# mklarqvist/StormBitmaps

Hardware: AMD Instinct MI355X
Metric: 64-bit bitmap words/s, XX^T upper-tri pairwise AND+popcount (10000x65536) (higher is better)
Workload: dtype u64 (bits as exact FP4 0/1 MFMA operands, f32 accumulate < 2^24); 1 GPU; STORM_contiguous_t N=10000 M=65536 dense draws=32768 seed=42 (BASELINE configs[1], README `benchmark 65536 10000`); entry_point=storm_hip_pairw_dense_launch == STORM_contig_pairw_intersect_cardinality_blocked, kernel_variant=4, work_items=13688

## Files before the change

### stormbitmaps_amd/csrc/storm_hip.hip

```cpp
#include "storm_hip_internal.h"

#include <chrono>

#include <algorithm>
#include <atomic>
#include <cstdarg>
#include <cstdlib>
#include <cstring>

namespace storm {

static thread_local char g_error[512] = "";

void set_error(const char* fmt, ...) {
    va_list ap;
    va_start(ap, fmt);
    vsnprintf(g_error, sizeof(g_error), fmt, ap);
    va_end(ap);
}

#define STORM_PAIR(A, B)                 \
    "v_and_b32 %[t], %[" A "], %[" B "]\n\t" \
    "s_nop 0\n\t"                        \
    "v_bcnt_u32_b32 %[acc], %[t], %[acc]\n\t"
// ... 605 lines not shown
        {"k2_max_run", &C::k2_max_run, RANGE, 0, 4096, 0, {},
         "k2_max_run out of range (0 = chosen by the list-scheduling estimate, 1..4096)"},
        {"k2_ring", &C::k2_ring, HOOK, 0, 0, 0, {}, nullptr, {}, nullptr, set_ring},
        {"k2_shadow_budget_mb", &C::k2_shadow_budget_mb, RANGE, 0, 1 << 22, 0, {}, "k2_shadow_budget_mb must be 0 (unbounded) .. 4194304",
         {}, nullptr, nullptr, drop_shadow},
        {"k2_tile_shape", &C::k2_tile_shape, SET, 0, 0, 0, {0, 1, 2, 3, 4, 5, 6, 16, 32},
         "k2_tile_shape must be 0 (chosen by the matrix), 5 (both operands as FP4 images in the LDS, 16x16x128 MFMAs), 1, 2 (bit operands inflated in registers), 3 / 4 (B as FP4 images in the LDS, 16x16x128 / 32x32x64 MFMAs), 6 (128 x 128 tiles, k-parts whose sums meet inside the launch), 16 or 32 (FP4 shadow)",
         {1, 16},
         "k2_tile_shape = 1 / 16 (tilebits_kernel, tile16_fp4_kernel) is a form of the tools build (`make probes`), not of the shipped library"},
        {"k2_ring_sync", &C::k2_ring_sync, BOOL},
        {"k2_wave_below", &C::k2_wave_below, RANGE, 0, 1 << 30, 0, {}, "k2_wave_below: 0 (never) .. 2^30 tiles of 256 x 256"},
        {"k2_part_slots", &C::k2_part_slots, RANGE, 0, 2, 0, {}, "k2_part_slots must be 0 (by the length of the segments), 1 or 2 per CU"},
        {"k2_part_min_chunks", &C::k2_part_min_chunks, RANGE, 1, 4096, 0, {}, "k2_part_min_chunks: 1 .. 4096 chunks of 512 bits"},
        {"k2_part_narrow", &C::k2_part_narrow, BOOL},
        {"k2_part_cost_diag", &C::k2_part_cost_diag, RANGE, 10, 100, 0, {}, "k2_part_cost_diag: 10 .. 100 percent of a full tile's chunk"},
        {"k2_ring_cost_diag", &C::k2_ring_cost_diag, RANGE, 5, 100, 0, {}, kCostText},
        {"k2_ring_cost_ragged", &C::k2_ring_cost_ragged, RANGE, 5, 100, 0, {}, kCostText},
        {"k2_tile_cost_diag", &C::k2_tile_cost_diag, RANGE, 5, 100, 0, {}, kCostText},
        {"k2_tile_cost_ragged", &C::k2_tile_cost_ragged, RANGE, 5, 100, 0, {}, kCostText},
        {"k2_strip_operands", &C::k2_strip_operands, RANGE, 0, 6, 0, {},
         "k2_strip_operands must be 0 (by size), 1 (bit operands, one item per workgroup), 2 (bit operands, one stream per workgroup), 3 (the same with a ring per wave), 4 (FP4 shadow), 5 (bit operands, FP4 image built in the LDS) or 6 (the same with 512-row A tiles, two halves behind one image)",
         {1, 3},
         "k2_strip_operands = 1 (stripbits_kernel) and 3 (bitwave_kernel) are forms of the tools build (`make probes`), not of the shipped library"},
        {"k2_shard_pairs", &C::k2_shard_pairs, BOOL},
        {"k2_matrix_pad", &C::k2_matrix_pad, HOOK, 0, 0, 0, {}, nullptr, {}, nullptr, set_matrix_pad},
        {"k2_fold_inline", &C::k2_fold_inline, HOOK, 0, 0, 0, {}, nullptr, {}, nullptr, set_fold_inline},
        {"k2_wave_ring", &C::k2_wave_ring, SET, 0, 0, 0, {0, 3, 4, 6, 8}, "k2_wave_ring must be 0 (by occupancy), 3, 4, 6 or 8"},
        {"k2_stream_max_rows", &C::k2_stream_max_rows, RANGE, 0, 1ll << 31, 0, {}, "k2_stream_max_rows must be 0 .. 2^31"},
        {"k2_stream_groups_per_cu", &C::k2_stream_groups_per_cu, RANGE, 0, 255, 0, {}, "k2_stream_groups_per_cu must be 0 (auto) .. 255"},
        {"k2_stream_min_piece", &C::k2_stream_min_piece, RANGE, 1, 4096, 0, {}, "%s must be 1..4096 stages"},
        {"k2_stream_min_run", &C::k2_stream_min_run, RANGE, 1, 4096, 0, {}, "%s must be 1..4096 stages"},
        {"k2_stream_w3_1", &C::k2_stream_w3_1, RANGE, 10, 1000, 0, {}, "%s must be 10..1000 percent of the first workgroup's share"},
        {"k2_stream_w3_2", &C::k2_stream_w3_2, RANGE, 10, 1000, 0, {}, "%s must be 10..1000 percent of the first workgroup's share"},
        {"k2_shape", &C::k2_shape, SET, 0, 0, 0, {16, 32}, "k2_shape must be 16 (16x16x128 MFMA) or 32 (32x32x64)", {32},
         "k2_shape = 32 (strip_fp4_kernel) is a form of the tools build (`make probes`), not of the shipped library"},
        {"keep_shadow", &C::keep_shadow, BOOL, 0, 0, 0, {}, nullptr, {}, nullptr, nullptr, drop_shadow},
        {"k2_matrix_parts", &C::k2_matrix_parts, BOOL},
        {"k2_matrix_min_part", &C::k2_matrix_min_part, RANGE, 4, 4096, 4, {},
         "k2_matrix_min_part: a multiple of 4 in 4 .. 4096 (stages of 128 bits)"},
        {"k2_matrix_split", &C::k2_matrix_split, BOOL},
        {"k2_pitch_pad", &C::k2_pitch_pad, RANGE, -1, 65536, 128, {}, "k2_pitch_pad must be -1 (auto) or a multiple of 128 in 0..65536"},
        {"k2_lds_pad", &C::k2_lds_pad, RANGE, 0, 120 * 1024, 0, {}, "k2_lds_pad must be 0..122880"},
        {"k2_persistent", &C::k2_persistent, BOOL, 0, 0, 0, {}, nullptr, {1},
         "k2_persistent (strip_fp4_kernel with work queues) is a form of the tools build (`make probes`), not of the shipped library"},
        {"k2_lpt_rounds", &C::k2_lpt_rounds, RANGE, 0, 63, 0, {}, "k2_lpt_rounds must be 0..63"},
        {"k2_tail_slices", &C::k2_tail_slices, RANGE, 0, 255, 0, {}, "k2_tail_slices must be 0..255"},
// ... 26 lines not shown
    }
    if (row->kind == OptionRow::HOOK) return row->hook(ctx, value);
    const auto among = [](const std::vector<int64_t>& set, int64_t v) { return std::find(set.begin(), set.end(), v) != set.end(); };
    const int64_t stored = row->kind == OptionRow::BOOL ? value != 0 : value;
    if ((row->kind == OptionRow::RANGE && (value < row->lo || value > row->hi || (row->step && value > 0 && value % row->step))) ||
        (row->kind == OptionRow::SET && !among(row->set, value))) {
        set_error(row->text, key);
        return STORM_HIP_EINVAL;
    }
    if (!kToolsBuild && among(row->tools_only, stored)) {
        set_error(row->tools_text, key);
        return STORM_HIP_EINVAL;
    }
    ctx->*(row->member) = (int)stored;
    if (row->after) row->after(ctx, value);
    return STORM_HIP_OK;
}

int64_t storm_hip_ctx_get_option(storm_hip_ctx_t* ctx, const char* key) {
    if (check_ctx(ctx) || !key) return -1;
    if (const OptionRow* row = find_option(key)) return ctx->*(row->member);
    if (!strcmp(key, "variant_used")) return ctx->variant_used;
    if (!strcmp(key, "k2_operands_used")) return ctx->k2_operands_used;
    if (!strcmp(key, "k2_tile_shape_used")) return ctx->k2_tile_shape_eff;
    if (!strcmp(key, "n_cus")) return ctx->n_cus;
    if (!strcmp(key, "probes_build") || !strcmp(key, "probes_built")) return kToolsBuild;
    return -1;
}

int storm_hip_kernel_time(storm_hip_ctx_t* ctx, double* sum_ms, uint64_t* launches) {
    if (check_ctx(ctx) || !sum_ms || !launches) return STORM_HIP_EINVAL;
    STORM_HIP_TRY(hipSetDevice(ctx->device));
    STORM_HIP_TRY(hipStreamSynchronize(ctx->stream));
    *sum_ms = 0.0;
    *launches = 0;
    for (size_t i = 0; i + 1 < ctx->kernel_events_used; i += 2) {
        float ms = 0.f;
        STORM_HIP_TRY(hipEventElapsedTime(&ms, ctx->kernel_events[i], ctx->kernel_events[i + 1]));
        *sum_ms += ms;
        ++*launches;
    }
    ctx->kernel_events_used = 0;
    return STORM_HIP_OK;
}

int storm_hip_debug_strip_trace(storm_hip_ctx_t* ctx, uint64_t* out, uint64_t capacity_items,
// ... 826 lines not shown
```

### stormbitmaps_amd/csrc/storm_hip_internal.h

```cpp
#pragma once

#include <hip/hip_runtime.h>

#include <algorithm>
#include <cstdint>
#include <cstdio>
#include <exception>
#include <cstring>
#include <new>
#include <optional>
#include <thread>
#include <utility>
#include <variant>
#include <vector>

#include "storm_hip.h"
#include "storm_hip_plan.h"

struct storm_hip_ctx_s;
typedef struct storm_hip_ctx_s storm_hip_ctx_t;
struct storm_hip_matrix_s;

namespace storm {

// ... 111 lines not shown
    uint64_t last_info[4] = {0, 0, 0, 0};
    uint64_t sparse_census[4] = {0, 0, 0, 0};
    uint64_t pass_report[4] = {0, 0, 0, 0};
    storm::DevBuf<uint8_t> d_x4;
    storm::DevBuf<void> d_items;
    std::variant<std::monostate, storm::TileSumRequest, storm::MatrixTilesRequest, storm::Tile128Request> items_key;
    uint32_t n_items = 0;
    storm::MatrixPlan matrix_plan;
    void* panel_lists = nullptr;
    hipStream_t copy_stream = nullptr;
    storm::DevBuf<storm::StripItem> d_strip_items;
    std::optional<storm::StripRequest> strip_key;
    uint32_t n_strip_items = 0;
    int k2_stages_per_item = 32;
    int k2_max_run = 0;
    int k2_ring = 4;
    int k2_shadow_budget_mb = 96 * 1024;
    int k2_strip_operands = 0;
    int k2_stream_max_rows = 8192;
    int k2_shard_pairs = 0;
    int k2_matrix_pad = -1;
    int k2_fold_inline = -1;
    int k2_operands_used = 4;
    int k2_tile_shape = 0;
    int k2_wave_below = 400;
    int k2_part_slots = 0;
    int k2_part_min_chunks = 8;
    int k2_part_narrow = 1;
    int k2_part_cost_diag = 80;
    uint32_t n_part_items = 0;
    storm::DevBuf<uint32_t> d_tickets;
    bool tickets_dirty = false;
    int k2_tile_shape_eff = 2;
    int k2_ring_sync = 0;
    int k2_ring_cost_diag = 78, k2_ring_cost_ragged = 40;
    int k2_tile_cost_diag = 63, k2_tile_cost_ragged = 30;
    int k2_shape = 16;
    int k2_persistent = 0;
    uint32_t strip_queue_base[8] = {0, 0, 0, 0, 0, 0, 0, 0};
    uint32_t strip_queue_count[8] = {0, 0, 0, 0, 0, 0, 0, 0};
    int keep_shadow = 0;
    uint64_t x4_key[4] = {0, 0, 0, 0};
    int k2_matrix_split = 1;
    int k2_matrix_parts = 0;
    storm::DevBuf<uint32_t> d_parts;
    int k2_matrix_min_part = 32;
// ... 21 lines not shown
    int k2_stream_w3_1 = 120, k2_stream_w3_2 = 60;
    int k2_wave_ring = 0;
    bool trace_is_stream = false;
    int k2_debug = 0;
};

namespace storm {
int launch_pairw_mfma(storm_hip_ctx_t* ctx, const storm_hip_matrix_s* m, uint32_t shard_rank,
                      uint32_t shard_count, uint64_t* d_total);
int launch_pairw_mfma_ranges(storm_hip_ctx_t* ctx, const uint64_t* X, uint64_t stride_words,
                             uint64_t n_rows_src, uint64_t n_rows_dst,
                             const std::vector<RowRange>& ranges, uint32_t shard_rank,
                             uint32_t shard_count, int strip_mode, uint64_t* d_total,
                             uint64_t shadow_generation = 0, uint32_t n_words_logical = 0);
int launch_pairw_bits_upload(storm_hip_ctx_t* ctx, storm_hip_matrix_s* m, const uint64_t* host_rows,
                             uint64_t src_stride_words, uint64_t* d_total);
int stage_check_lists(const storm_hip_stage_s* stage, const std::vector<uint64_t>& ltable);
int stage_gather_lists(storm_hip_ctx_t* ctx, storm_hip_stage_s* stage, const std::vector<uint64_t>& ltable, uint16_t* d_lists,
                       uint64_t** d_table);
int strip_operands_of(const storm_hip_ctx_t* ctx);
int launch_pairw_bits_ranges(storm_hip_ctx_t* ctx, const uint8_t* X, uint64_t pitch_bytes,
                             const std::vector<RowRange>& ranges, uint32_t n_kslices2, uint32_t shard_rank,
                             uint32_t shard_count, uint64_t* d_total, bool slots_hold_sums = false,
                             uint32_t a_tile = 256u);
static inline uint64_t ranges_word_pairs(const std::vector<RowRange>& ranges, uint64_t words, uint32_t shard_count) {
    uint64_t pairs = 0;
    for (const RowRange& rg : ranges) {
        const uint64_t n = rg.r1 - rg.r0, a = rg.a_end ? std::min(rg.a_end, rg.r1) - rg.r0 : n;
        pairs += a * (a - (a != 0)) / 2 + a * (n - a);
    }
    return pairs * words / (shard_count ? shard_count : 1);
}
int launch_pairw_matrix(storm_hip_ctx_t* ctx, const storm_hip_matrix_s* m, int op, uint32_t* d_out,
                        uint64_t ld, uint64_t band_row0 = 0, uint64_t band_rows = ~0ull,
                        bool sync = true);
int launch_pairw_lag_matrix(storm_hip_ctx_t* ctx, const storm_hip_matrix_s* m, int op, uint64_t max_lag, uint64_t band_row0,
                            uint64_t band_rows, uint32_t* d_out, uint64_t ld, bool sync);
int launch_pairw_dosage_matrix(storm_hip_ctx_t* ctx, const storm_hip_matrix_s* m, uint32_t* d_out, uint64_t ld, bool sync);
int launch_square_mfma(storm_hip_ctx_t* ctx, const storm_hip_matrix_s* a,
                       const storm_hip_matrix_s* b, uint64_t* d_total);
int launch_square_matrix(storm_hip_ctx_t* ctx, const storm_hip_matrix_s* a,
                         const storm_hip_matrix_s* b, int op, uint32_t* d_out, uint64_t ld,
                         bool sync = true);
int launch_row_counts(storm_hip_ctx_t* ctx, const storm_hip_matrix_s* m, uint32_t* d_counts);
int launch_similarity_finish(storm_hip_ctx_t* ctx, void* d_io, uint64_t ld, uint64_t n_rows, uint64_t n_cols,
                             const uint32_t* d_counts_rows, const uint32_t* d_counts_cols, int triangle, int measure,
                             uint64_t n_bits);
// ... 127 lines not shown
```

### stormbitmaps_amd/csrc/storm_hip_mfma.hip

```cpp
#include "storm_hip_internal.h"

#include <algorithm>
#include <chrono>
#include <cstring>
#include <exception>
#include <type_traits>
#include <utility>

namespace storm {

#ifdef STORM_HIP_PROBES
__device__ unsigned long long g_clock_probe[4];
#define STORM_CLOCK_BEGIN()                                  \
    const uint64_t ck_t0 = __builtin_amdgcn_s_memtime();     \
    const uint64_t ck_r0 = __builtin_amdgcn_s_memrealtime()
#define STORM_CLOCK_END()                                                                           \
    do {                                                                                            \
        if (threadIdx.x == 0) {                                                                     \
            atomicAdd(&g_clock_probe[0], (unsigned long long)(__builtin_amdgcn_s_memtime() - ck_t0)); \
            atomicAdd(&g_clock_probe[1], (unsigned long long)(__builtin_amdgcn_s_memrealtime() - ck_r0)); \
            atomicAdd(&g_clock_probe[2], 1ull);                                                     \
        }                                                                                           \
    } while (0)
#else
// ... 462 lines not shown
[[maybe_unused]] constexpr int kSb16BitStage = kStripBRows * 64;
constexpr uint32_t kSb16ImgBytes = kSb16ImgRing * kStripStageBytes;
constexpr uint32_t kSb16Mask = 0x22222222u;

__device__ __forceinline__ v4i sb16_inflate(v4i w, uint32_t rot) {
    v4i e;
    e.x = (int)(__builtin_amdgcn_alignbit((uint32_t)w.x, (uint32_t)w.x, rot) & kSb16Mask);
    e.y = (int)(__builtin_amdgcn_alignbit((uint32_t)w.y, (uint32_t)w.y, rot) & kSb16Mask);
    e.z = (int)(__builtin_amdgcn_alignbit((uint32_t)w.z, (uint32_t)w.z, rot) & kSb16Mask);
    e.w = (int)(__builtin_amdgcn_alignbit((uint32_t)w.w, (uint32_t)w.w, rot) & kSb16Mask);
    return e;
}

#define STORM_SB16_WAVES 4
#define STORM_SB16_NAME strip16_bits_kernel
#include "strip16_bits_kernel.inc"
#undef STORM_SB16_WAVES
#undef STORM_SB16_NAME
#define STORM_SB16_WAVES 8
#define STORM_SB16_NAME strip16_bits2_kernel
#include "strip16_bits_kernel.inc"
#undef STORM_SB16_WAVES
#undef STORM_SB16_NAME

[[maybe_unused]] constexpr int kT16Ring = 4;
constexpr int kT16RowBytes = 128;
[[maybe_unused]] constexpr int kT16StageBytes = kTile * kT16RowBytes;

#ifdef STORM_HIP_PROBES
#include "../../tools/probes/tile16_fp4.hip"
#endif

[[maybe_unused]] constexpr int kTbThreads = 256;
constexpr int kTbRing = 4;
constexpr int kTbRowBytes = 64;
constexpr int kTbImageBytes = kTile * kTbRowBytes;
constexpr int kTbStageBytes = 2 * kTbImageBytes;

template <int C>
__device__ __forceinline__ v4i tb_inflate(v4i w) {
    typedef unsigned v4u __attribute__((ext_vector_type(4)));
    if constexpr (C == 3) return (v4i)(((v4u)w >> 1u) & 0x44444444u);
    else return w & (int)(0x11111111u << C);
}
template <int C>
__device__ __forceinline__ int tb_scale() {
// ... 1469 lines not shown
                           ctx->d_bitfirst.d,
                           ctx->d_bitfirst.d + 2 * ((size_t)ctx->n_bit_groups + 1),
                           ctx->d_bitfirst.d + ((size_t)ctx->n_bit_groups + 1), ctx->d_slots,
                           reinterpret_cast<unsigned long long*>(d_total), ctx->d_trace);
    } else
#endif
        hipLaunchKernelGGL(bitstream_kernel<false>, grid, block, 0, ctx->stream,
                           reinterpret_cast<const uint8_t*>(X), pitch, ctx->d_bitsegs.d,
                           ctx->d_bitfirst.d,
                           ctx->d_bitfirst.d + 2 * ((size_t)ctx->n_bit_groups + 1),
                           ctx->d_bitfirst.d + ((size_t)ctx->n_bit_groups + 1), ctx->d_slots,
                           reinterpret_cast<unsigned long long*>(d_total), (unsigned long long*)nullptr);
    kernel_time_mark(ctx);
    STORM_HIP_TRY(hipGetLastError());
    return STORM_HIP_OK;
}

#ifdef STORM_HIP_PROBES
#include "../../tools/probes/bitwave_launch.hip"
#endif

int launch_pairw_bits_ranges(storm_hip_ctx_t* ctx, const uint8_t* X, uint64_t pitch,
                             const std::vector<RowRange>& ranges, uint32_t n_kslices2, uint32_t shard_rank,
                             uint32_t shard_count, uint64_t* d_total, bool slots_hold_sums, uint32_t a_tile) {
    if (pitch * (uint64_t)kStripBRows >= (1ull << 32)) {
        set_error("K2b: rows of %llu bytes are beyond the strips' 32-bit DMA offsets", (unsigned long long)pitch);
        return STORM_HIP_EINVAL;
    }
    ctx->n_items = 0;
    ctx->items_key = std::monostate{};
    if (int rc = ensure_strip_items(ctx, ranges, n_kslices2, shard_rank, shard_count, a_tile, 2))
        return rc;
    const uint32_t n_strip = ctx->n_strip_items;
    const uint32_t waves = a_tile / (uint32_t)kStripBRows;
    ctx->k2_operands_used = waves == 8u ? 6 : 5;
    if (n_strip > 0) {
        ctx->pass_report[0] |= STORM_HIP_RAN_BIT_STRIPS;
        ctx->pass_report[1] += ranges_word_pairs(ranges, (uint64_t)n_kslices2 * 4u, shard_count);
    }
    ctx->last_info[0] = n_strip;
    ctx->last_info[1] = ctx->k2_stages_per_item;
    ctx->last_info[2] = 1;
    ctx->last_info[3] = 0;
    const uint32_t fold_slots = n_strip <= 4096u ? 256u : (uint32_t)kSlots;
    const bool fold_wanted = ctx->k2_fold_inline > 0 || (ctx->k2_fold_inline < 0 && n_strip <= 4096u);
    const uint64_t arrivals_per_slot = (uint64_t)n_strip * (uint64_t)waves / (uint64_t)fold_slots + 1u;
    const uint64_t wave_sum_max = 64ull * (4096ull * 64ull + 256ull) * 256ull;
    const bool fold_inline = fold_wanted && !slots_hold_sums && n_strip > 0 && arrivals_per_slot < 65535u &&
                             arrivals_per_slot * wave_sum_max < (1ull << 48);
    if (n_strip > 0) {
        kernel_time_mark(ctx);
        if (waves == 8u)
            hipLaunchKernelGGL(strip16_bits2_kernel, dim3(n_strip), dim3(512), (size_t)ctx->k2_lds_pad,
                               ctx->stream, X, pitch, ctx->d_strip_items.d, ctx->d_slots,
                               fold_inline ? reinterpret_cast<unsigned long long*>(d_total) : nullptr, fold_slots);
        else
            hipLaunchKernelGGL(strip16_bits_kernel, dim3(n_strip), dim3(kStripThreads), (size_t)ctx->k2_lds_pad,
                               ctx->stream, X, pitch, ctx->d_strip_items.d, ctx->d_slots,
                               fold_inline ? reinterpret_cast<unsigned long long*>(d_total) : nullptr, fold_slots);
        kernel_time_mark(ctx);
        STORM_HIP_TRY(hipGetLastError());
    }
    return fold_inline ? STORM_HIP_OK : launch_fold_slots(ctx, d_total);
}

static int launch_pairw_bits(storm_hip_ctx_t* ctx, const storm_hip_matrix_s* m, uint32_t shard_rank,
                             uint32_t shard_count, int operands, uint64_t* d_total) {
    const uint64_t pitch = m->stride_words * 8;
    const uint64_t n_rows4 = (m->n_rows + kStripATile - 1) / kStripATile * kStripATile;
    if (n_rows4 > m->n_rows_pad || pitch * (uint64_t)kStripBRows >= (1ull << 32)) {
        set_error("K2sb: matrix of %llu rows (%llu allocated) x %llu bytes per row is outside the bit-operand strips' reach",
                  (unsigned long long)m->n_rows, (unsigned long long)m->n_rows_pad, (unsigned long long)pitch);
        return STORM_HIP_EINVAL;
    }
    std::vector<RowRange> ranges;
    if (m->n_rows > 1) ranges.push_back({0, m->n_rows});
    const uint32_t n_kslices = (m->n_words + 7u) / 8u;
    if (operands == 2)
        return launch_pairw_bitstream(ctx, m->d, pitch, ranges, n_kslices, shard_rank, shard_count, d_total);
#ifdef STORM_HIP_PROBES
    if (operands == 3)
        return launch_pairw_bitwave(ctx, m->d, pitch, ranges, n_kslices, shard_rank, shard_count, d_total);
#endif
    ctx->n_items = 0;
    ctx->items_key = std::monostate{};
    if (operands == 5 || operands == 6)
        return launch_pairw_bits_ranges(ctx, reinterpret_cast<const uint8_t*>(m->d), pitch, ranges, n_kslices * 2u,
                                        shard_rank, shard_count, d_total, false, operands == 6 ? 512u : (uint32_t)kStripATile);
    if (int rc = ensure_strip_items(ctx, ranges, n_kslices, shard_rank, shard_count, (uint32_t)kStripATile))
        return rc;
#ifndef STORM_HIP_PROBES
    set_error("k2_strip_operands = 1 (stripbits_kernel) is in the tools build only (`make probes`)");
    return STORM_HIP_EINVAL;
#else
    const uint32_t n_strip = ctx->n_strip_items;
    if (n_strip > 0) {
        kernel_time_mark(ctx);
        hipLaunchKernelGGL(stripbits_kernel, dim3(n_strip), dim3(kStripThreads), 0, ctx->stream,
                           reinterpret_cast<const uint8_t*>(m->d), pitch,
                           ctx->d_strip_items.d, ctx->d_slots);
        kernel_time_mark(ctx);
        STORM_HIP_TRY(hipGetLastError());
    }
    ctx->last_info[0] = n_strip;
    ctx->last_info[1] = ctx->k2_stages_per_item;
    ctx->last_info[2] = 1;
    ctx->last_info[3] = 0;
    return launch_fold_slots(ctx, d_total);
#endif
}

// ... 15 lines not shown
    const uint64_t tiles = (m->n_rows + kStripATile - 1) / kStripATile;
    if (tiles * kStripATile > m->n_rows_pad || pitch * (uint64_t)kStripBRows >= (1ull << 32) || m->n_rows < 2) {
        set_error("pairw_dense_upload: matrix outside the bit-operand strips' reach");
        return STORM_HIP_EINVAL;
    }
    if (!ctx->copy_stream) STORM_HIP_TRY(hipStreamCreateWithFlags(&ctx->copy_stream, hipStreamNonBlocking));
    if (!ctx->panel_lists) ctx->panel_lists = new std::vector<PanelList>();
    auto& lists = *static_cast<std::vector<PanelList>*>(ctx->panel_lists);
    if (lists.empty()) lists.resize(1);
    if (!lists[0].landed) STORM_HIP_TRY(hipEventCreateWithFlags(&lists[0].landed, hipEventDisableTiming));
    STORM_HIP_TRY(hipEventRecord(lists[0].landed, ctx->stream));
    STORM_HIP_TRY(hipStreamWaitEvent(ctx->copy_stream, lists[0].landed, 0));
    std::vector<uint64_t> first_tile;
    {
        const uint64_t n = std::max<uint64_t>(1, std::min<uint64_t>(8, tiles / 4));
        for (uint64_t p = 0; p <= n; ++p) first_tile.push_back(tiles * p / n);
    }
    const uint64_t n_panels = first_tile.size() - 1;
    const uint32_t n_kslices2 = 2u * ((m->n_words + 7u) / 8u);
    if (lists.size() < n_panels) lists.resize(n_panels);
    ctx->pass_report[0] |= STORM_HIP_RAN_BIT_STRIPS;
    ctx->pass_report[1] += ranges_word_pairs({{0, m->n_rows}}, (uint64_t)n_kslices2 * 4u, 1);
    ctx->k2_operands_used = 5;
    uint64_t n_total = 0;
    for (uint64_t p = 0; p < n_panels; ++p) {
        const uint64_t t0 = first_tile[p], t1 = first_tile[p + 1];
        if (t0 >= t1) continue;
        const uint64_t row0 = t0 * kStripATile, row1 = std::min<uint64_t>(m->n_rows, t1 * kStripATile);
        PanelList& l = lists[p];
        if (!l.landed) STORM_HIP_TRY(hipEventCreateWithFlags(&l.landed, hipEventDisableTiming));
        STORM_HIP_TRY(hipMemcpy2DAsync(m->d + row0 * m->stride_words, pitch, host_rows + row0 * src_stride_words,
                                       src_stride_words * 8, (size_t)m->n_words * 8, row1 - row0, hipMemcpyHostToDevice,
                                       ctx->copy_stream));
        STORM_HIP_TRY(hipEventRecord(l.landed, ctx->copy_stream));
        StripOptions po = strip_options_of(ctx, 2);
        po.max_run = 128;
        po.shard_pairs = po.persistent = po.one_slice_probe = 0;
        RowRange rg{0, row1};
        rg.back_from = row0;
        const std::vector<RowRange> panel = {rg};
        const StripRequest rq = strip_request(po, panel, n_kslices2, 0, 1, (uint32_t)kStripATile);
        if (!l.d || !(l.key == rq)) {
            l.key.reset();
            std::vector<StripItem> items;
            uint32_t qb[8], qc[8];
            plan_strips(rq, panel, items, qb, qc);
// ... 72 lines not shown
```

### stormbitmaps_amd/csrc/storm_hip_plan.cpp

```cpp
#include "storm_hip_plan.h"

#include <algorithm>
#include <cmath>
#include <cstdio>
#include <cstdlib>
#include <chrono>
#include <exception>

#include "storm_hip.h"

namespace storm {

bool timing_env() {
    static const bool on = getenv("STORM_HIP_TIMING") != nullptr;
    return on;
}

uint64_t ranges_hash(const std::vector<RowRange>& ranges) {
    uint64_t h = 1469598103934665603ull;
    for (const RowRange& r : ranges) {
        h = (h ^ r.r0) * 1099511628211ull;
        h = (h ^ r.r1) * 1099511628211ull;
        h = (h ^ r.a_end) * 1099511628211ull;
        h = (h ^ r.back_from) * 1099511628211ull;
// ... 1092 lines not shown
        set_error("lag_plan: bad arguments");
        return STORM_HIP_EINVAL;
    }
    try {
        Tile128Plan plan;
        const uint64_t end = std::min(n_rows, band_row0 + std::min(band_rows ? band_rows : n_rows, n_rows));
        const uint32_t lag = (uint32_t)std::min<uint64_t>(max_lag, n_rows - 1);
        if (band_row0 < end && lag)
            plan_tile128({(uint32_t)(band_row0 / kThTile), (uint32_t)((end + kThTile - 1) / kThTile), 0u,
                          (uint32_t)((n_rows + kThTile - 1) / kThTile), 1u, (n_words + 7u) / 8u * 4u, n_cus, slots_per_cu,
                          min_chunks, diag_cost_pct, 1u, lag, kThWeightBits}, &plan);
        return export_part_items("lag_plan", plan, out, capacity_items, n_items);
    } catch (const std::exception& e) {
        set_error("lag_plan: %s", e.what());
        return STORM_HIP_ENOMEM;
    }
}

extern "C" int storm_hip_strip_plan3(uint64_t n_rows, uint32_t n_words, uint32_t shard_rank,
                                     uint32_t shard_count, int form, int pair_space, int max_run, int tail_run,
                                     int tail_slices, int lpt_rounds, uint32_t n_cus, uint32_t* out,
                                     uint64_t capacity_items, uint64_t* n_items, int* run_chosen) {
    using namespace storm;
    if (!n_items || shard_count == 0 || shard_rank >= shard_count || n_words == 0 || (form != 0 && form != 1) ||
        max_run < 0 || max_run > 4096 || tail_run < 1 || tail_run > 4096 || tail_slices < 0 || tail_slices > 255 ||
        lpt_rounds < 0 || lpt_rounds > 63 || n_cus == 0) {
        set_error("strip_plan: bad arguments");
        return STORM_HIP_EINVAL;
    }
    try {
        const uint32_t n_kslices = form == 0 ? (n_words + 3u) / 4u : 2u * ((n_words + 7u) / 8u);
        std::vector<RowRange> ranges;
        if (n_rows > 1) ranges.push_back({0, n_rows});
        std::vector<StripItem> items;
        uint32_t qb[8], qc[8];
        StripOptions o;
        o.max_run = max_run;
        o.tail_run = tail_run;
        o.tail_slices = tail_slices;
        o.lpt_rounds = lpt_rounds;
        o.shard_pairs = pair_space != 0;
        o.n_cus = (int)n_cus;
        o.xcd_group = form == 0 ? 1 : 2;
        plan_strips(strip_request(o, ranges, n_kslices, shard_rank, shard_count, (uint32_t)kStripATile), ranges, items, qb, qc,
                    run_chosen);
        *n_items = items.size();
        if (out)
            for (uint64_t i = 0; i < std::min<uint64_t>(capacity_items, items.size()); ++i) {
                out[i * 5 + 0] = items[i].a_row0;
                out[i * 5 + 1] = items[i].diag;
                out[i * 5 + 2] = items[i].j0;
                out[i * 5 + 3] = items[i].j1;
                out[i * 5 + 4] = items[i].ks;
            }
    } catch (const std::exception& e) {
        set_error("strip_plan: %s", e.what());
        return STORM_HIP_ENOMEM;
    }
    return STORM_HIP_OK;
}

extern "C" int storm_hip_strip_plan2(uint64_t n_rows, uint32_t n_words, uint32_t shard_rank,
                                     uint32_t shard_count, int form, int pair_space, uint32_t* out,
                                     uint64_t capacity_items, uint64_t* n_items) {
    const storm::StripOptions d;
    return storm_hip_strip_plan3(n_rows, n_words, shard_rank, shard_count, form, pair_space, d.max_run, d.tail_run,
                                 d.tail_slices, d.lpt_rounds, (uint32_t)d.n_cus, out, capacity_items, n_items, nullptr);
}
// ... 48 lines not shown
```

### stormbitmaps_amd/csrc/storm_hip_plan.h

```cpp
#pragma once

#include <cstdint>
#include <cstring>
#include <type_traits>
#include <utility>
#include <vector>

namespace storm {

void set_error(const char* fmt, ...);
bool timing_env();

template <class T>
inline bool same_request(const T& a, const T& b) {
    static_assert(std::has_unique_object_representations_v<T>, "a request struct with padding cannot be compared with memcmp");
    return !memcmp(&a, &b, sizeof(T));
}

constexpr int kChunkWords = 64;

constexpr int kTile = 256;
constexpr int kStageBytes = 64;
constexpr uint32_t kGroupStages = 32;

struct MfmaItem {
    uint16_t I, J;
    uint32_t stage0;
    uint32_t n_stages;
};
static_assert(sizeof(MfmaItem) == 12, "read by device code");

constexpr uint32_t kOwnSlices = 4;
constexpr int kStripRowBytes = 128;
constexpr int kStripBRows = 64;
constexpr int kStripWaves = 4;
constexpr int kStripATile = 64 * kStripWaves;

struct StripItem {
    uint32_t a_row0;
    uint32_t diag;
    uint32_t j0, j1;
    uint32_t ks;
};
static_assert(sizeof(StripItem) == 20, "read by device code");

struct BitSeg {
    uint32_t a_blk;
    uint32_t ks;
    uint32_t b_first;
    uint32_t n_b;
    uint32_t range_b0;
    uint32_t range_nb;
    uint32_t flags;
    uint32_t pad;
};
static_assert(sizeof(BitSeg) == 32, "read by device code");
constexpr uint32_t kBsDiag = 1u;
constexpr uint32_t kBsMaxStages = 8192;

// ... 237 lines not shown
```

### stormbitmaps_amd/csrc/storm_hip_sparse.hip

```cpp
#include "storm_hip_internal.h"

#include <algorithm>
#include <atomic>
#include <chrono>
#include <cstring>
#include <exception>
#include <memory>
#include <thread>

using namespace storm;

namespace storm {
__global__ void warm_sparse_kernel() {}
void warm_sparse_code(hipStream_t stream) { hipLaunchKernelGGL(warm_sparse_kernel, dim3(1), dim3(64), 0, stream); }
}


constexpr uint64_t kPoolPitchDefault = 1024;

struct storm_hip_sparse_s : storm::ArenaColumns, storm::ProbeWork {
    uint64_t* d_pool = nullptr;
    uint64_t pitch = kPoolPitchDefault;
    uint32_t* d_probe_elems = nullptr;
    uint16_t* d_probe_pos16 = nullptr;
// ... 1333 lines not shown
        RowRange rg = s->cols[e];
        if (use_probe[e]) {
            if (s->col_list0[e] == rg.r0) continue;
            rg.a_end = s->col_list0[e];
        }
        if (rg.r1 - rg.r0 > 1) {
            ranges.push_back(rg);
            rows_needed = std::max(rows_needed, rg.r1);
        }
    }
    if (s->n_probe_launch > 0) {
        ctx->pass_report[0] |= STORM_HIP_RAN_LIST_PROBE;
        ctx->pass_report[2] += s->probe_lookups_launch;
        ctx->pass_report[3] = kProbeRows;
        const bool probe_folds = ranges.empty() && ctx->k2_fold_inline != 0 && s->n_probe_launch <= 16384u &&
                                 s->probe_lookups_launch < (1ull << 38);
        if (int rc = launch_probe(ctx, s, shard_rank, shard_count,
                                  probe_folds ? reinterpret_cast<unsigned long long*>(d_result) : nullptr))
            return rc;
        if (probe_folds) {
            ctx->last_info[0] = 0;
            ctx->last_info[3] = s->n_probe_cols_launch;
            ctx->k2_operands_used = 5;
            return STORM_HIP_OK;
        }
    }
    if (rows_needed > s->pool_rows_ready)
        if (int rc = ensure_full_pool(ctx, s)) return rc;
    const uint64_t rows_dst = (rows_needed + 511) / 512 * 512;
    if (variant == 4 && strip_operands_of(ctx) == 5 && ctx->k2_debug == 0 && !ctx->k2_persistent &&
        rows_dst <= s->pool_rows_ready + 512) {
        if (int rc = launch_pairw_bits_ranges(ctx, reinterpret_cast<const uint8_t*>(s->d_pool), s->pitch * 8ull,
                                              ranges, kBlockWords / 4u, shard_rank, shard_count,
                                              d_result, s->n_probe_launch > 0))
            return rc;
    } else if (int rc = launch_pairw_mfma_ranges(ctx, s->d_pool, s->pitch, s->pool_rows_ready + 512,
                                                 std::max<uint64_t>(rows_dst, 512), ranges,
                                                 shard_rank, shard_count, variant == 5 ? 2 : variant == 4 ? 1 : 0,
                                                 d_result))
        return rc;
    ctx->last_info[3] = s->n_probe_cols_launch;
    return STORM_HIP_OK;
    });
}

int storm_hip_sparse_last_census(storm_hip_ctx_t* ctx, uint64_t out[4]) {
// ... 7 lines not shown
```

### stormbitmaps_amd/dist.py

```python
from __future__ import annotations

import os
from typing import Callable, Tuple


def rank_world() -> Tuple[int, int, int]:
    return (int(os.environ.get("RANK", "0")), int(os.environ.get("WORLD_SIZE", "1")),
            int(os.environ.get("LOCAL_RANK", "0")))


def free_port() -> int:
    import socket
    with socket.socket() as sock:
        sock.bind(("127.0.0.1", 0))
        return sock.getsockname()[1]


def init_process_group(backend: str):
    import torch.distributed as dist
    if not dist.is_initialized():
        rank, world, _ = rank_world()
        os.environ.setdefault("MASTER_ADDR", "127.0.0.1")
        if "MASTER_PORT" not in os.environ:
            if world > 1:
# ... 8 lines not shown
               max_run: int = 0, tail_run: int = 32, tail_slices: int = 3, lpt_rounds: int = 6, n_cus: int = 256,
               return_run: bool = False):
    import ctypes as C

    import numpy as np

    from . import _lib
    lib = _lib.load()
    n = C.c_uint64(0)
    run = C.c_int(0)
    args = (n_rows, n_words, rank, world, form, pair_space, max_run, tail_run, tail_slices, lpt_rounds, n_cus)
    _lib.check(lib.storm_hip_strip_plan3(*args, None, 0, C.byref(n), C.byref(run)), "storm_hip_strip_plan3")
    out = np.zeros((int(n.value), 5), dtype=np.uint32)
    if n.value:
        _lib.check(lib.storm_hip_strip_plan3(*args, out.ctypes.data_as(C.c_void_p), n.value, C.byref(n), C.byref(run)),
                   "storm_hip_strip_plan3")
    return (out, int(run.value)) if return_run else out


def slice_columns(mat, ks: int, form: int = 1):
    import numpy as np
    if form == 0:
        return np.ascontiguousarray(mat[:, 4 * ks:4 * ks + 4])
    c = ks // 2
    mask = np.uint64(0xCCCCCCCCCCCCCCCC if ks & 1 else 0x3333333333333333)
    return np.ascontiguousarray(mat[:, 8 * c:8 * c + 8] & mask)


def stream_plan(n_rows: int, n_words: int, rank: int = 0, world: int = 1, n_cus: int = 256):
    import ctypes as C

    import numpy as np

    from . import _lib
    lib = _lib.load()
    n, g = C.c_uint64(0), C.c_uint32(0)
    _lib.check(lib.storm_hip_stream_plan(n_rows, n_words, rank, world, n_cus, None, 0, C.byref(n), C.byref(g)),
               "storm_hip_stream_plan")
    out = np.zeros((int(n.value), 8), dtype=np.uint32)
    if n.value:
        _lib.check(lib.storm_hip_stream_plan(n_rows, n_words, rank, world, n_cus, out.ctypes.data_as(C.c_void_p),
                                             n.value, C.byref(n), C.byref(g)), "storm_hip_stream_plan")
    return out, int(g.value)


def matrix_plan(n_rows_a: int, n_words: int, n_rows_b: int = 0, band_row0: int = 0, band_rows: int = 0, n_cus: int = 256,
# ... 67 lines not shown
```

Measured before the change: 135000 billion words/s.

## Add 128-rows-per-wave strip kernel with 512-row A tiles on 128-bit slices

Adds a new strip16_rows_kernel in which each of four waves holds 128 A rows as inflated FP4 operands and streams B strips through a three-slot LDS image ring on 128-bit k-slices. It is chosen by rule for large single-shard matrices. Each B image fetched from LDS now feeds twice as many MFMAs, which is meant to cut LDS traffic and image building per MFMA. The cost is higher register pressure, coarser 512-row tiles and an eight-XCD grouping in the planner, which may worsen load balance on the diagonal.

```diff
diff --git a/stormbitmaps_amd/csrc/storm_hip.hip b/stormbitmaps_amd/csrc/storm_hip.hip
--- a/stormbitmaps_amd/csrc/storm_hip.hip
+++ b/stormbitmaps_amd/csrc/storm_hip.hip
@@ -651,6 +651,8 @@
          "k2_strip_operands must be 0 (by size), 1 (bit operands, one item per workgroup), 2 (bit operands, one stream per workgroup), 3 (the same with a ring per wave), 4 (FP4 shadow), 5 (bit operands, FP4 image built in the LDS) or 6 (the same with 512-row A tiles, two halves behind one image)",
          {1, 3},
          "k2_strip_operands = 1 (stripbits_kernel) and 3 (bitwave_kernel) are forms of the tools build (`make probes`), not of the shipped library"},
+        {"k2_strip_rows", &C::k2_strip_rows, SET, 0, 0, 0, {0, 64, 128},
+         "k2_strip_rows must be 0 (by rule), 64 (64 A rows per wave, 256-row A tiles) or 128 (128 A rows per wave on 128-bit slices, 512-row A tiles)"},
         {"k2_shard_pairs", &C::k2_shard_pairs, BOOL},
         {"k2_matrix_pad", &C::k2_matrix_pad, HOOK, 0, 0, 0, {}, nullptr, {}, nullptr, set_matrix_pad},
         {"k2_fold_inline", &C::k2_fold_inline, HOOK, 0, 0, 0, {}, nullptr, {}, nullptr, set_fold_inline},
@@ -723,6 +725,7 @@
     if (const OptionRow* row = find_option(key)) return ctx->*(row->member);
     if (!strcmp(key, "variant_used")) return ctx->variant_used;
     if (!strcmp(key, "k2_operands_used")) return ctx->k2_operands_used;
+    if (!strcmp(key, "k2_strip_rows_used")) return ctx->k2_strip_rows_used;
     if (!strcmp(key, "k2_tile_shape_used")) return ctx->k2_tile_shape_eff;
     if (!strcmp(key, "n_cus")) return ctx->n_cus;
     if (!strcmp(key, "probes_build") || !strcmp(key, "probes_built")) return kToolsBuild;
diff --git a/stormbitmaps_amd/csrc/storm_hip_internal.h b/stormbitmaps_amd/csrc/storm_hip_internal.h
--- a/stormbitmaps_amd/csrc/storm_hip_internal.h
+++ b/stormbitmaps_amd/csrc/storm_hip_internal.h
@@ -157,6 +157,8 @@
     int k2_matrix_pad = -1;
     int k2_fold_inline = -1;
     int k2_operands_used = 4;
+    int k2_strip_rows = 0;
+    int k2_strip_rows_used = 64;
     int k2_tile_shape = 0;
     int k2_wave_below = 400;
     int k2_part_slots = 0;
@@ -224,7 +226,8 @@
 int launch_pairw_bits_ranges(storm_hip_ctx_t* ctx, const uint8_t* X, uint64_t pitch_bytes,
                              const std::vector<RowRange>& ranges, uint32_t n_kslices2, uint32_t shard_rank,
                              uint32_t shard_count, uint64_t* d_total, bool slots_hold_sums = false,
-                             uint32_t a_tile = 256u);
+                             uint32_t a_tile = 256u,
+                             bool rows128 = false);
 static inline uint64_t ranges_word_pairs(const std::vector<RowRange>& ranges, uint64_t words, uint32_t shard_count) {
     uint64_t pairs = 0;
     for (const RowRange& rg : ranges) {
diff --git a/stormbitmaps_amd/csrc/storm_hip_mfma.hip b/stormbitmaps_amd/csrc/storm_hip_mfma.hip
--- a/stormbitmaps_amd/csrc/storm_hip_mfma.hip
+++ b/stormbitmaps_amd/csrc/storm_hip_mfma.hip
@@ -508,6 +508,23 @@
 #include "strip16_bits_kernel.inc"
 #undef STORM_SB16_WAVES
 #undef STORM_SB16_NAME
+
+constexpr uint32_t kSr16SliceBytes = 16;
+constexpr uint32_t kSr16PerTile = kStripRowsATile / kStripBRows;
+constexpr uint32_t kSr16StageBytes = kStripBRows * 64;
+constexpr uint32_t kSr16ImgBytes = 3 * kSr16StageBytes;
+constexpr uint32_t kSr16BitRing = 3;
+constexpr uint32_t kSr16BitStage = 4 * 256;
+
+__device__ __forceinline__ v4i sr16_inflate(uint32_t w) {
+    v4i e;
+    e.x = (int)(__builtin_amdgcn_alignbit(w, w, 31u) & kSb16Mask);
+    e.y = (int)(w & kSb16Mask);
+    e.z = (int)(__builtin_amdgcn_alignbit(w, w, 1u) & kSb16Mask);
+    e.w = (int)(__builtin_amdgcn_alignbit(w, w, 2u) & kSb16Mask);
+    return e;
+}
+#include "strip16_rows_kernel.inc"
 
 [[maybe_unused]] constexpr int kT16Ring = 4;
 constexpr int kT16RowBytes = 128;
@@ -2023,21 +2040,26 @@
 
 int launch_pairw_bits_ranges(storm_hip_ctx_t* ctx, const uint8_t* X, uint64_t pitch,
                              const std::vector<RowRange>& ranges, uint32_t n_kslices2, uint32_t shard_rank,
-                             uint32_t shard_count, uint64_t* d_total, bool slots_hold_sums, uint32_t a_tile) {
+                             uint32_t shard_count, uint64_t* d_total, bool slots_hold_sums, uint32_t a_tile, bool rows128) {
     if (pitch * (uint64_t)kStripBRows >= (1ull << 32)) {
         set_error("K2b: rows of %llu bytes are beyond the strips' 32-bit DMA offsets", (unsigned long long)pitch);
         return STORM_HIP_EINVAL;
     }
     ctx->n_items = 0;
     ctx->items_key = std::monostate{};
-    if (int rc = ensure_strip_items(ctx, ranges, n_kslices2, shard_rank, shard_count, a_tile, 2))
+    if (rows128 && a_tile != kStripRowsATile) {
+        set_error("K2b: the 128-rows-per-wave form takes A tiles of 512 rows");
+        return STORM_HIP_EINVAL;
+    }
+    if (int rc = ensure_strip_items(ctx, ranges, n_kslices2, shard_rank, shard_count, a_tile, rows128 ? (int)kStripRowsXcdGroup : 2))
         return rc;
     const uint32_t n_strip = ctx->n_strip_items;
-    const uint32_t waves = a_tile / (uint32_t)kStripBRows;
+    const uint32_t waves = rows128 ? 4u : a_tile / (uint32_t)kStripBRows;
     ctx->k2_operands_used = waves == 8u ? 6 : 5;
+    ctx->k2_strip_rows_used = rows128 ? 128 : 64;
     if (n_strip > 0) {
         ctx->pass_report[0] |= STORM_HIP_RAN_BIT_STRIPS;
-        ctx->pass_report[1] += ranges_word_pairs(ranges, (uint64_t)n_kslices2 * 4u, shard_count);
+        ctx->pass_report[1] += ranges_word_pairs(ranges, (uint64_t)n_kslices2 * (rows128 ? 2u : 4u), shard_count);
     }
     ctx->last_info[0] = n_strip;
     ctx->last_info[1] = ctx->k2_stages_per_item;
@@ -2046,12 +2068,17 @@
     const uint32_t fold_slots = n_strip <= 4096u ? 256u : (uint32_t)kSlots;
     const bool fold_wanted = ctx->k2_fold_inline > 0 || (ctx->k2_fold_inline < 0 && n_strip <= 4096u);
     const uint64_t arrivals_per_slot = (uint64_t)n_strip * (uint64_t)waves / (uint64_t)fold_slots + 1u;
-    const uint64_t wave_sum_max = 64ull * (4096ull * 64ull + 256ull) * 256ull;
+    const uint64_t wave_sum_max = rows128 ? 128ull * (4096ull * 64ull + 512ull) * 128ull
+                                          : 64ull * (4096ull * 64ull + 256ull) * 256ull;
     const bool fold_inline = fold_wanted && !slots_hold_sums && n_strip > 0 && arrivals_per_slot < 65535u &&
                              arrivals_per_slot * wave_sum_max < (1ull << 48);
     if (n_strip > 0) {
         kernel_time_mark(ctx);
-        if (waves == 8u)
+        if (rows128)
+            hipLaunchKernelGGL(strip16_rows_kernel, dim3(n_strip), dim3(256), (size_t)ctx->k2_lds_pad,
+                               ctx->stream, X, pitch, ctx->d_strip_items.d, ctx->d_slots,
+                               fold_inline ? reinterpret_cast<unsigned long long*>(d_total) : nullptr, fold_slots);
+        else if (waves == 8u)
             hipLaunchKernelGGL(strip16_bits2_kernel, dim3(n_strip), dim3(512), (size_t)ctx->k2_lds_pad,
                                ctx->stream, X, pitch, ctx->d_strip_items.d, ctx->d_slots,
                                fold_inline ? reinterpret_cast<unsigned long long*>(d_total) : nullptr, fold_slots);
@@ -2063,6 +2090,14 @@
         STORM_HIP_TRY(hipGetLastError());
     }
     return fold_inline ? STORM_HIP_OK : launch_fold_slots(ctx, d_total);
+}
+
+static bool strip_rows128_by_rule(const storm_hip_matrix_s* m, uint32_t shard_count) {
+    return shard_count == 1 && m->n_rows >= 2048 && m->n_words >= 1024;
+}
+static bool strip_rows128(const storm_hip_ctx_t* ctx, const storm_hip_matrix_s* m, uint32_t shard_count) {
+    if (ctx->k2_strip_rows == 64 || ctx->k2_strip_operands == 6 || (m->n_rows + kStripRowsATile - 1) / kStripRowsATile * kStripRowsATile > m->n_rows_pad) return false;
+    return ctx->k2_strip_rows == 128 || strip_rows128_by_rule(m, shard_count);
 }
 
 static int launch_pairw_bits(storm_hip_ctx_t* ctx, const storm_hip_matrix_s* m, uint32_t shard_rank,
@@ -2085,9 +2120,12 @@
 #endif
     ctx->n_items = 0;
     ctx->items_key = std::monostate{};
+    if (operands == 5 && strip_rows128(ctx, m, shard_count))
+        return launch_pairw_bits_ranges(ctx, reinterpret_cast<const uint8_t*>(m->d), pitch, ranges, strip_rows_kslices(m->n_words),
+                                        shard_rank, shard_count, d_total, false, kStripRowsATile, true);
     if (operands == 5 || operands == 6)
         return launch_pairw_bits_ranges(ctx, reinterpret_cast<const uint8_t*>(m->d), pitch, ranges, n_kslices * 2u,
-                                        shard_rank, shard_count, d_total, false, operands == 6 ? 512u : (uint32_t)kStripATile);
+                                        shard_rank, shard_count, d_total, false, operands == 6 ? 512u : (uint32_t)kStripATile, false);
     if (int rc = ensure_strip_items(ctx, ranges, n_kslices, shard_rank, shard_count, (uint32_t)kStripATile))
         return rc;
 #ifndef STORM_HIP_PROBES
@@ -2149,6 +2187,7 @@
     ctx->pass_report[0] |= STORM_HIP_RAN_BIT_STRIPS;
     ctx->pass_report[1] += ranges_word_pairs({{0, m->n_rows}}, (uint64_t)n_kslices2 * 4u, 1);
     ctx->k2_operands_used = 5;
+    ctx->k2_strip_rows_used = 64;
     uint64_t n_total = 0;
     for (uint64_t p = 0; p < n_panels; ++p) {
         const uint64_t t0 = first_tile[p], t1 = first_tile[p + 1];
diff --git a/stormbitmaps_amd/csrc/storm_hip_plan.cpp b/stormbitmaps_amd/csrc/storm_hip_plan.cpp
--- a/stormbitmaps_amd/csrc/storm_hip_plan.cpp
+++ b/stormbitmaps_amd/csrc/storm_hip_plan.cpp
@@ -1138,14 +1138,14 @@
                                      int tail_slices, int lpt_rounds, uint32_t n_cus, uint32_t* out,
                                      uint64_t capacity_items, uint64_t* n_items, int* run_chosen) {
     using namespace storm;
-    if (!n_items || shard_count == 0 || shard_rank >= shard_count || n_words == 0 || (form != 0 && form != 1) ||
+    if (!n_items || shard_count == 0 || shard_rank >= shard_count || n_words == 0 || form < 0 || form > 2 ||
         max_run < 0 || max_run > 4096 || tail_run < 1 || tail_run > 4096 || tail_slices < 0 || tail_slices > 255 ||
         lpt_rounds < 0 || lpt_rounds > 63 || n_cus == 0) {
         set_error("strip_plan: bad arguments");
         return STORM_HIP_EINVAL;
     }
     try {
-        const uint32_t n_kslices = form == 0 ? (n_words + 3u) / 4u : 2u * ((n_words + 7u) / 8u);
+        const uint32_t n_kslices = form == 0 ? (n_words + 3u) / 4u : form == 1 ? 2u * ((n_words + 7u) / 8u) : strip_rows_kslices(n_words);
         std::vector<RowRange> ranges;
         if (n_rows > 1) ranges.push_back({0, n_rows});
         std::vector<StripItem> items;
@@ -1157,9 +1157,9 @@
         o.lpt_rounds = lpt_rounds;
         o.shard_pairs = pair_space != 0;
         o.n_cus = (int)n_cus;
-        o.xcd_group = form == 0 ? 1 : 2;
-        plan_strips(strip_request(o, ranges, n_kslices, shard_rank, shard_count, (uint32_t)kStripATile), ranges, items, qb, qc,
-                    run_chosen);
+        o.xcd_group = form == 0 ? 1 : form == 1 ? 2 : (int)kStripRowsXcdGroup;
+        plan_strips(strip_request(o, ranges, n_kslices, shard_rank, shard_count, form == 2 ? kStripRowsATile : (uint32_t)kStripATile),
+                    ranges, items, qb, qc, run_chosen);
         *n_items = items.size();
         if (out)
             for (uint64_t i = 0; i < std::min<uint64_t>(capacity_items, items.size()); ++i) {
diff --git a/stormbitmaps_amd/csrc/storm_hip_plan.h b/stormbitmaps_amd/csrc/storm_hip_plan.h
--- a/stormbitmaps_amd/csrc/storm_hip_plan.h
+++ b/stormbitmaps_amd/csrc/storm_hip_plan.h
@@ -35,6 +35,9 @@
 constexpr int kStripBRows = 64;
 constexpr int kStripWaves = 4;
 constexpr int kStripATile = 64 * kStripWaves;
+constexpr uint32_t kStripRowsATile = 512;
+constexpr uint32_t kStripRowsXcdGroup = 8;
+inline uint32_t strip_rows_kslices(uint32_t n_words) { return (n_words + 1u) / 2u; }
 
 struct StripItem {
     uint32_t a_row0;
diff --git a/stormbitmaps_amd/csrc/storm_hip_sparse.hip b/stormbitmaps_amd/csrc/storm_hip_sparse.hip
--- a/stormbitmaps_amd/csrc/storm_hip_sparse.hip
+++ b/stormbitmaps_amd/csrc/storm_hip_sparse.hip
@@ -1379,6 +1379,7 @@
             ctx->last_info[0] = 0;
             ctx->last_info[3] = s->n_probe_cols_launch;
             ctx->k2_operands_used = 5;
+            ctx->k2_strip_rows_used = 64;
             return STORM_HIP_OK;
         }
     }
diff --git a/stormbitmaps_amd/csrc/strip16_rows_kernel.inc b/stormbitmaps_amd/csrc/strip16_rows_kernel.inc
--- /dev/null
+++ b/stormbitmaps_amd/csrc/strip16_rows_kernel.inc
@@ -0,0 +1,291 @@
+__global__ __launch_bounds__(256, 4) void strip16_rows_kernel(
+    const uint8_t* __restrict__ X, uint64_t row_bytes, const StripItem* __restrict__ items,
+    unsigned long long* __restrict__ slots, unsigned long long* __restrict__ out, uint32_t fold_slots) {
+    __shared__ __attribute__((aligned(1024))) uint8_t lds_raw[kSr16ImgBytes + kSr16BitRing * kSr16BitStage];
+
+    constexpr uint32_t kW = 4u;
+    STORM_CLOCK_BEGIN();
+    const uint32_t tid = threadIdx.x;
+    const uint32_t lane = tid & 63u;
+    const uint32_t wave = __builtin_amdgcn_readfirstlane(tid >> 6);
+    const StripItem it = items[blockIdx.x];
+    const uint64_t kbyte = (uint64_t)it.ks * (uint64_t)kSr16SliceBytes;
+    const uint32_t D = it.diag ? kSr16PerTile : 0u;
+    const uint32_t T = D + (it.j1 - it.j0);
+    const uint32_t cslot = (3u - D % 3u) % 3u;
+
+    const uint32_t lds_base =
+        (uint32_t)(uintptr_t)(__attribute__((address_space(3))) uint8_t*)&lds_raw[0];
+    const uint32_t pr = wave * 16u + (lane >> 2);
+    const uint32_t goff0 = pr * (uint32_t)row_bytes + (lane & 3u) * 4u;
+    const uint32_t bits_rd = lds_base + kSr16ImgBytes + wave * 256u + lane * 4u;
+    const uint32_t img_wr = lds_base + pr * 64u + (((lane & 3u) ^ ((0x78u >> (2u * ((pr >> 2) & 3u))) & 3u)) * 16u);
+
+    auto issue = [&](uint32_t s, uint32_t slot) {
+        const uint32_t sc = min(s, T - 1u);
+        const uint32_t blk = sc < D ? it.a_row0 / (uint32_t)kStripBRows + sc : it.j1 - 1u - (sc - D);
+        const uint8_t* base = X + (uint64_t)(blk * (uint32_t)kStripBRows) * row_bytes + kbyte;
+        const __amdgpu_buffer_rsrc_t rsrc =
+            __builtin_amdgcn_make_buffer_rsrc(const_cast<uint8_t*>(base), 0, -1, 0x00020000);
+        __builtin_amdgcn_raw_ptr_buffer_load_lds(
+            rsrc, (lptr_t)(lds_raw + kSr16ImgBytes + slot * kSr16BitStage + wave * 256u), 4,
+            (int)goff0, 0, 0, 0);
+    };
+
+    v4i a[8];
+    {
+        const uint8_t* ap = X + (uint64_t)(it.a_row0 + wave * 64u + (lane & 15u)) * row_bytes + kbyte +
+                            (lane >> 4) * 4u;
+        uint32_t aw[8];
+#pragma unroll
+        for (int m = 0; m < 8; ++m)
+            aw[m] = *reinterpret_cast<const uint32_t*>(ap + (uint64_t)((m & 3) * 16 + (m >> 2) * 256) * row_bytes);
+        issue(0u, cslot);
+        issue(1u, (cslot + 1u) % 3u);
+        issue(2u, (cslot + 2u) % 3u);
+#pragma unroll
+        for (int m = 0; m < 8; ++m) a[m] = sr16_inflate(aw[m]);
+    }
+
+    v4f acc[8][2];
+#pragma unroll
+    for (int m = 0; m < 8; ++m)
+#pragma unroll
+        for (int n = 0; n < 2; ++n) acc[m][n] = v4f{};
+
+    const uint32_t boff = lds_base + (lane & 15u) * 64u + (((lane >> 4) ^ ((0x78u >> (2u * ((lane & 15u) >> 2))) & 3u)) * 16u);
+
+#pragma unroll
+    for (int m = 0; m < 8; ++m) asm volatile("" ::"v"(a[m]));
+
+#define STORM_FETCH16(dst, img, j)                                                        \
+    asm volatile("ds_read_b128 %0, %1 offset:%2"                                          \
+                 : "=&v"(dst)                                                             \
+                 : "v"(boff), "n"((img) + (j) * 16 * 64))
+#define STORM_FETCH16V(dst, img, j)                                                       \
+    asm volatile("ds_read_b128 %0, %1 offset:%2"                                          \
+                 : "=&v"(dst)                                                             \
+                 : "v"(boff + (img)), "n"((j) * 16 * 64))
+#define STORM_MUL1(m, j, frag)                                                            \
+    acc[m][(j) & 1] = __builtin_amdgcn_mfma_scale_f32_16x16x128_f8f6f4(                   \
+        v8i{a[m].x, a[m].y, a[m].z, a[m].w, 0, 0, 0, 0},                                  \
+        v8i{frag.x, frag.y, frag.z, frag.w, 0, 0, 0, 0}, acc[m][(j) & 1], 4, 4, 0, 0, 0, 0)
+#define STORM_MUL16(j, frag)                                                              \
+    _Pragma("unroll") for (int m = 0; m < 8; ++m) STORM_MUL1(m, j, frag)
+#define STORM_LGKM_STR(n) asm volatile("s_waitcnt lgkmcnt(" #n ")" ::: "memory")
+#define STORM_LGKM(n)    \
+    STORM_LGKM_STR(n);   \
+    __builtin_amdgcn_sched_barrier(0)
+#define STORM_VM2()                                         \
+    asm volatile("s_waitcnt vmcnt(2)" ::: "memory");        \
+    __builtin_amdgcn_sched_barrier(0)
+
+    uint32_t wb = 0;
+    auto build_image = [&](uint32_t s) {
+        uint32_t slot = (s + cslot) % 3u;
+        asm volatile("" : "+s"(slot));
+        asm volatile("ds_read_b32 %0, %1" : "=&v"(wb) : "v"(bits_rd + slot * kSr16BitStage));
+        STORM_LGKM(0);
+        const v4i e = sr16_inflate(wb);
+        asm volatile("ds_write_b128 %0, %1" ::"v"(img_wr + slot * kSr16StageBytes), "v"(e) : "memory");
+        __builtin_amdgcn_sched_barrier(0);
+    };
+
+    asm volatile("s_waitcnt lgkmcnt(0)" ::: "memory");
+    STORM_VM2();
+    build_image(0u);
+    STORM_LGKM(0);
+    issue(3u, cslot);
+    STORM_VM2();
+    build_image(1u);
+
+    v4i b0 = {}, b1 = {}, b2 = {};
+    uint32_t t = 0;
+    if (D != 0u) {
+#define STORM_SR16_MASK(m, n)                                                             \
+    _Pragma("unroll") for (int r = 0; r < 4; ++r) acc[m][n][r] = r < tri ? acc[m][n][r] : 0.0f;
+#define STORM_SR16_WHOLE(base, j)                                                         \
+    _Pragma("unroll") for (int i = 0; i < 4; ++i) {                                       \
+        STORM_MUL1((base) + i, j, b0);                                                    \
+        STORM_MUL1((base) + i, (j) + 1, b1);                                              \
+    }
+#define STORM_SR16_OWN01(base)                                                            \
+    STORM_MUL1((base) + 0, 0, b0);                                                        \
+    STORM_SR16_MASK((base) + 0, 0)                                                        \
+    STORM_MUL1((base) + 0, 1, b1);                                                        \
+    STORM_MUL1((base) + 1, 1, b1);                                                        \
+    STORM_SR16_MASK((base) + 1, 1)
+#define STORM_SR16_OWN23(base)                                                            \
+    STORM_MUL1((base) + 0, 2, b0);                                                        \
+    STORM_MUL1((base) + 1, 2, b0);                                                        \
+    STORM_MUL1((base) + 2, 2, b0);                                                        \
+    STORM_SR16_MASK((base) + 2, 0)                                                        \
+    STORM_MUL1((base) + 0, 3, b1);                                                        \
+    STORM_MUL1((base) + 1, 3, b1);                                                        \
+    STORM_MUL1((base) + 2, 3, b1);                                                        \
+    STORM_MUL1((base) + 3, 3, b1);                                                        \
+    STORM_SR16_MASK((base) + 3, 1)
+#define STORM_SR16_HEAD()                                                                 \
+    STORM_LGKM(0);                                                  \
+    __builtin_amdgcn_s_barrier();     \
+    issue(t + 4u, (t + 1u + cslot) % 3u);                                                 \
+    STORM_VM2();                                                         \
+    build_image(t + 2u);                                                                  \
+    uint32_t sb = ((t + cslot) % 3u) * kSr16StageBytes;                                   \
+    asm volatile("" : "+s"(sb))
+#define STORM_SR16_PAIR(j)                                                                \
+    __builtin_amdgcn_sched_barrier(0);                                                    \
+    STORM_FETCH16V(b0, sb, j);                                                            \
+    STORM_FETCH16V(b1, sb, (j) + 1);                                                      \
+    STORM_LGKM(0)
+#pragma unroll 1
+        for (; t < wave; ++t) {
+            STORM_SR16_HEAD();
+        }
+        {
+            STORM_SR16_HEAD();
+            const uint32_t lane_d = __builtin_amdgcn_mbcnt_hi(~0u, __builtin_amdgcn_mbcnt_lo(~0u, 0u));
+            const int tri = (int)(lane_d & 15u) - (int)(4u * (lane_d >> 4));
+            STORM_SR16_PAIR(0);
+            STORM_SR16_OWN01(0)
+            STORM_SR16_PAIR(2);
+            STORM_SR16_OWN23(0)
+            ++t;
+        }
+#pragma unroll 1
+        for (; t < wave + 4u; ++t) {
+            STORM_SR16_HEAD();
+            STORM_SR16_PAIR(0);
+            STORM_SR16_WHOLE(0, 0)
+            STORM_SR16_PAIR(2);
+            STORM_SR16_WHOLE(0, 2)
+        }
+        {
+            STORM_SR16_HEAD();
+            const uint32_t lane_d = __builtin_amdgcn_mbcnt_hi(~0u, __builtin_amdgcn_mbcnt_lo(~0u, 0u));
+            const int tri = (int)(lane_d & 15u) - (int)(4u * (lane_d >> 4));
+            STORM_SR16_PAIR(0);
+            STORM_SR16_WHOLE(0, 0)
+            STORM_SR16_OWN01(4)
+            STORM_SR16_PAIR(2);
+            STORM_SR16_WHOLE(0, 2)
+            STORM_SR16_OWN23(4)
+            ++t;
+        }
+#pragma unroll 1
+        for (; t < kSr16PerTile; ++t) {
+            STORM_SR16_HEAD();
+            STORM_SR16_PAIR(0);
+            STORM_SR16_WHOLE(0, 0)
+            STORM_SR16_WHOLE(4, 0)
+            STORM_SR16_PAIR(2);
+            STORM_SR16_WHOLE(0, 2)
+            STORM_SR16_WHOLE(4, 2)
+        }
+        __builtin_amdgcn_sched_barrier(0);
+#undef STORM_SR16_PAIR
+#undef STORM_SR16_HEAD
+#undef STORM_SR16_OWN23
+#undef STORM_SR16_OWN01
+#undef STORM_SR16_WHOLE
+#undef STORM_SR16_MASK
+    }
+#define STORM_SR16_BODY(I, fa, fb, fc)                                                                      \
+    {                                                                                                       \
+        issue(t + 4u, ((I) + 1) % 3);              \
+        STORM_VM2();                                               \
+        asm volatile("ds_read_b32 %0, %1 offset:%2" : "=&v"(wb) : "v"(bits_rd), "n"((((I) + 2) % 3) * kSr16BitStage)); \
+        v4i e;                                                                                              \
+        STORM_FETCH16(fc, (I) * kSr16StageBytes, 2); STORM_LGKM(3); STORM_MUL16(0, fa); __builtin_amdgcn_sched_barrier(0); \
+        STORM_FETCH16(fa, (I) * kSr16StageBytes, 3); STORM_LGKM(2);       \
+        e = sr16_inflate(wb); STORM_MUL16(1, fb); __builtin_amdgcn_sched_barrier(0);                        \
+        asm volatile("ds_write_b128 %0, %1 offset:%2" ::"v"(img_wr), "v"(e), "n"((((I) + 2) % 3) * kSr16StageBytes) : "memory"); \
+        STORM_FETCH16(fb, (((I) + 1) % 3) * kSr16StageBytes, 0); STORM_LGKM(3); STORM_MUL16(2, fc); __builtin_amdgcn_sched_barrier(0); \
+        STORM_FETCH16(fc, (((I) + 1) % 3) * kSr16StageBytes, 1); STORM_LGKM(2); STORM_MUL16(3, fa); __builtin_amdgcn_sched_barrier(0); \
+        ++t;                                                                                                \
+        if (t >= T) break;                                                                                  \
+        __builtin_amdgcn_s_barrier();                                                                       \
+    }
+    if (t < T) {
+        STORM_LGKM(0);
+        __builtin_amdgcn_s_barrier();
+        STORM_FETCH16(b0, 0, 0);
+        STORM_FETCH16(b1, 0, 1);
+        for (;;) {
+            STORM_SR16_BODY(0, b0, b1, b2)
+            STORM_SR16_BODY(1, b1, b2, b0)
+            STORM_SR16_BODY(2, b2, b0, b1)
+        }
+        STORM_LGKM(0);
+    }
+    asm volatile("s_waitcnt vmcnt(0)" ::: "memory");
+    asm volatile("" ::"v"(b0), "v"(b1), "v"(b2), "v"(wb));
+#undef STORM_SR16_BODY
+#undef STORM_VM2
+#undef STORM_FETCH16V
+#undef STORM_FETCH16
+#undef STORM_MUL16
+#undef STORM_MUL1
+#undef STORM_LGKM
+#undef STORM_LGKM_STR
+
+    STORM_CLOCK_END();
+    uint64_t mine = 0;
+#pragma unroll
+    for (int m = 0; m < 8; ++m) {
+        uint32_t part = 0;
+#pragma unroll
+        for (int n = 0; n < 2; ++n)
+#pragma unroll
+            for (int r = 0; r < 4; ++r) part += (uint32_t)acc[m][n][r];
+        mine += part;
+    }
+#pragma unroll
+    for (int o = 32; o > 0; o >>= 1) mine += __shfl_down(mine, o, 64);
+    const uint32_t lane_e = __builtin_amdgcn_mbcnt_hi(~0u, __builtin_amdgcn_mbcnt_lo(~0u, 0u));
+    const uint32_t tid_e = wave * 64u + lane_e;
+    if (out == nullptr) {
+        if (lane_e == 0 && mine != 0)
+            atomicAdd(&slots[(blockIdx.x * kW + wave) & (kSlots - 1)],
+                      (unsigned long long)mine);
+        return;
+    }
+    if (lane_e == 0)
+        atomicAdd(&slots[(blockIdx.x * kW + wave) & (fold_slots - 1u)],
+                  (unsigned long long)mine + (1ull << 48));
+    if (blockIdx.x != gridDim.x - 1u) return;
+    const unsigned long long expected = (unsigned long long)gridDim.x * (unsigned long long)kW;
+    unsigned long long* wsum = reinterpret_cast<unsigned long long*>(lds_raw);
+    unsigned long long total = 0;
+    for (;;) {
+        unsigned long long cnt = 0, sum = 0;
+        for (uint32_t i = tid_e; i < fold_slots; i += (kW * 64u)) {
+            const unsigned long long v = __hip_atomic_load(&slots[i], __ATOMIC_RELAXED, __HIP_MEMORY_SCOPE_AGENT);
+            cnt += v >> 48;
+            sum += v & ((1ull << 48) - 1ull);
+        }
+#pragma unroll
+        for (int o = 32; o > 0; o >>= 1) {
+            cnt += __shfl_down(cnt, o, 64);
+            sum += __shfl_down(sum, o, 64);
+        }
+        __syncthreads();
+        if (lane_e == 0) {
+            wsum[wave] = cnt;
+            wsum[kW + wave] = sum;
+        }
+        __syncthreads();
+        cnt = 0;
+        total = 0;
+#pragma unroll
+        for (uint32_t w = 0; w < kW; ++w) {
+            cnt += wsum[w];
+            total += wsum[kW + w];
+        }
+        if (cnt == expected) break;
+        if (fold_slots > (kW * 64u)) __builtin_amdgcn_s_sleep(8);
+    }
+    for (uint32_t i = tid_e; i < fold_slots; i += (kW * 64u))
+        __hip_atomic_store(&slots[i], 0ull, __ATOMIC_RELAXED, __HIP_MEMORY_SCOPE_AGENT);
+    if (tid_e == 0) out[0] = total;
+}
diff --git a/stormbitmaps_amd/dist.py b/stormbitmaps_amd/dist.py
--- a/stormbitmaps_amd/dist.py
+++ b/stormbitmaps_amd/dist.py
@@ -54,6 +54,8 @@
     import numpy as np
     if form == 0:
         return np.ascontiguousarray(mat[:, 4 * ks:4 * ks + 4])
+    if form == 2:
+        return np.ascontiguousarray(mat[:, 2 * ks:2 * ks + 2])
     c = ks // 2
     mask = np.uint64(0xCCCCCCCCCCCCCCCC if ks & 1 else 0x3333333333333333)
     return np.ascontiguousarray(mat[:, 8 * c:8 * c + 8] & mask)
```

New measurement: 142000 billion words/s, median of 6. 1.05x the previous value.
